# iris-ua/iris_lama

Measured on AMD Instinct MI355X. Metric: particle-scans/sec, higher is better.
Workload: dtype f64; 1 GPU; PFSlam2D 30 particles, 1080-beam synthetic corridor log (SURVEY.md 8(d)), res 0.05 m, patch 32, l2_max 0.5, GN+Cauchy(0.15), seed 42; particles=30, beams=1080, parallelism=particle-shard x1

## Files before the change

include/lama_hip.h:

```cpp
#ifndef LAMA_HIP_H
#define LAMA_HIP_H

#include <stdint.h>

#ifdef __cplusplus
extern "C" {
#endif

#define LAMA_HIP_OK 0
#define LAMA_HIP_E_INVALID (-1)
#define LAMA_HIP_E_HIP (-2)
#define LAMA_HIP_E_WINDOW (-3)
#define LAMA_HIP_E_CAPACITY (-4)
#define LAMA_HIP_E_STATE (-5)
#define LAMA_HIP_E_NUMERIC (-6)

typedef struct lama_hip_ctx lama_hip_ctx;

typedef struct lama_hip_cfg {
    uint32_t particles;
    double resolution;
    uint32_t patch_size;
    double l2_max;
    double meas_sigma;
    uint32_t max_iter;
    double truncated_ray;
    double truncated_range;
    int32_t device;
    uint32_t window_patches;
    uint32_t dm_patch_capacity;
    uint32_t occ_patch_capacity;
    uint32_t queue_capacity;
    uint32_t profile;
    uint32_t active_capacity;
    uint32_t sequential_raycast;
    uint32_t brushfire_mode;
    uint32_t brushfire_waves;
    uint32_t occupancy_policy;
    uint32_t ray_rule;
    uint32_t solver_strategy;
} lama_hip_cfg;

void lama_hip_default_cfg(lama_hip_cfg* cfg);

int32_t lama_hip_device_count(int32_t* count);

int32_t lama_hip_ctx_create(const lama_hip_cfg* cfg, lama_hip_ctx** out);
void lama_hip_ctx_destroy(lama_hip_ctx* ctx);
const char* lama_hip_last_error(const lama_hip_ctx* ctx);

int32_t lama_hip_pf_init(lama_hip_ctx* ctx, const double* pts_xyz, uint32_t n,
                         const double* sensor_origin3, const double* sensor_quat_wxyz,
                         const double* pose0);

int32_t lama_hip_pf_set_poses(lama_hip_ctx* ctx, const double* poses);
int32_t lama_hip_pf_get_poses(lama_hip_ctx* ctx, double* poses);

int32_t lama_hip_pf_scan_match(lama_hip_ctx* ctx, const double* pts_xyz, uint32_t n,
                               const double* sensor_origin3, const double* sensor_quat_wxyz,
                               double* poses_out, double* loglik_out, int32_t* iters_out);

int32_t lama_hip_pf_resample(lama_hip_ctx* ctx, const int32_t* sample_idx);

int32_t lama_hip_pf_update_maps(lama_hip_ctx* ctx, const double* pts_xyz, uint32_t n,
                                const double* sensor_origin3, const double* sensor_quat_wxyz);

#define LAMA_HIP_MAP_DISTANCE 0
#define LAMA_HIP_MAP_OCCUPANCY 1
int32_t lama_hip_pf_map_patches(lama_hip_ctx* ctx, uint32_t particle, int32_t kind, uint32_t* num_patches);
int32_t lama_hip_pf_download_map(lama_hip_ctx* ctx, uint32_t particle, int32_t kind, uint32_t cap,
                                 uint64_t* patch_ids, uint8_t* cells, uint64_t* masks, uint32_t* num_patches);

int32_t lama_hip_pf_upload_map(lama_hip_ctx* ctx, uint32_t particle, int32_t kind, uint32_t num_patches,
                               const uint64_t* patch_ids, const uint8_t* cells, const uint64_t* masks);

int32_t lama_hip_pf_update_maps_begin(lama_hip_ctx* ctx, const double* pts_xyz, uint32_t n,
// ... 128 lines not shown
```

iris_lama_amd/csrc/lama_hip.hip:

```cpp
#include "../../include/lama_hip.h"

#include <hip/hip_runtime.h>

#include <algorithm>
#include <cmath>
#include <cstdio>
#include <cstdlib>
#include <cstring>
#include <map>
#include <memory>
#include <mutex>
#include <string>
#include <vector>

#include "lama_kernels.h"
#include "lama_pgo.h"
#include "lama_map_build.h"
#include "lama_match_batch.h"
#include "../host/pgo_pattern.hpp"

using namespace lama_dev;

namespace {

// ... 151 lines not shown
    DevBuf<uint8_t> d_early; DevBuf<uint32_t> d_elist;
    Stream stream3; Event ev_alloc, ev_go, ev_early;
    bool early_ok = false;
    uint32_t early_candidates = 0;
    std::vector<double> h_ll; bool ll_valid = false;
    PinVec<uint32_t> h_hlist; DevBuf<uint32_t> d_hlist;
    uint32_t early_on = 1;
    uint32_t early_min_count = 1024;
    Stream stream2; Event ev_route, ev_heavy;
    uint32_t route_min_count = 64, route_min_events = 48, route_percent = 150, route_cap = 64;
    bool route_forced = false; uint32_t num_cus = 256;
    bool debug_tail = false, debug_window = false;
    uint32_t big_stage_pad = 0;
    DevBuf<uint64_t> d_act; DevBuf<uint32_t> d_act_count;
    DevBuf<lama_dev::RayRec> d_rrec; DevBuf<uint64_t> d_rbbox; DevBuf<lama_dev::RayChunk> d_rchunk;
    int32_t* d_err = nullptr;
    DevBuf<double> d_pts; uint32_t last_n = 0;
    PinVec<uint64_t> h_stats;
    PinVec<double> h_tfs, h_pts;
    PinVec<int32_t> h_err;
    PinVec<uint32_t> h_slow_n;
    DevBuf<double> d_tfs;
    double* d_loglik = nullptr; int32_t* d_iters = nullptr;
    DevBuf<uint8_t> d_results;
    size_t results_bytes = 0, status_off = 0, status_bytes = 0;
    PinVec<uint8_t> h_status;
    PinVec<uint8_t> h_results;
    DevBuf<int32_t> d_oldcounts;
    DevBuf<double> d_mb_pts, d_mb_tfs; DevBuf<uint32_t> d_mb_offs; DevBuf<lama_dev::MbRay> d_mb_rays;
    DevBuf<uint32_t> d_mb_table, d_mb_off, d_mb_list, d_mb_bins; DevBuf<int32_t> d_mb_slot; DevBuf<uint64_t> d_mb_meta;
    PinVec<double> h_mb_tfs; PinVec<uint32_t> h_mb_offs; PinVec<uint64_t> h_mb_meta;
    DevBuf<double> d_bposes, d_bout;
    DevBuf<double> d_msb_f64; DevBuf<uint32_t> d_msb_u32;
    PinVec<double> h_msb_f64; PinVec<uint32_t> h_msb_u32;

    double scan_reach = 0.0;
    uint32_t visit_bound = 0;
    DevBuf<uint32_t> d_scalar;
    DevBuf<lama_dev::ShipDesc> d_ship_desc; DevBuf<uint8_t> d_ship_heads;
    PinVec<lama_dev::ShipDesc> h_ship_desc; PinVec<uint8_t> h_ship_heads;
    uint32_t* d_guard = nullptr;
    Affine last_mtf; uint32_t last_first = 0, last_count = 0;
    bool last_guarded = false;
    int recover_depth = 0;
    int64_t mbx0 = 0, mbx1 = 0, mby0 = 0, mby1 = 0; bool mb_valid = false;
    bool unguarded_retry = false;
// ... 844 lines not shown
}

int32_t lama_hip_device_count(int32_t* count)
{
    int n = 0;
    hipError_t e = hipGetDeviceCount(&n);
    if (count) *count = (e == hipSuccess) ? n : 0;
    return e == hipSuccess ? LAMA_HIP_OK : LAMA_HIP_E_HIP;
}

const char* lama_hip_last_error(const lama_hip_ctx* ctx) { return ctx ? ctx->error.c_str() : "null context"; }

int32_t lama_hip_ctx_create(const lama_hip_cfg* cfg_in, lama_hip_ctx** out)
{
    if (!cfg_in || !out) return LAMA_HIP_E_INVALID;
    *out = nullptr;
    lama_hip_cfg cfg = *cfg_in;
    if (cfg.window_patches == 0) cfg.window_patches = 128;
    if (cfg.dm_patch_capacity == 0) cfg.dm_patch_capacity = 128;
    if (cfg.occ_patch_capacity == 0) cfg.occ_patch_capacity = 128;
    if (cfg.queue_capacity == 0) cfg.queue_capacity = 32768;
    if (cfg.active_capacity == 0) cfg.active_capacity = 8192;
    if (cfg.active_capacity > 8192) cfg.active_capacity = 8192;
    if (cfg.brushfire_mode > 1 || cfg.brushfire_waves > 2) return LAMA_HIP_E_INVALID;
    if (cfg.particles == 0 || cfg.patch_size != 32 || !(cfg.resolution > 0) || cfg.window_patches > (uint32_t)LAMA_HIP_MAX_WINDOW ||
        (cfg.window_patches & 7) || cfg.dm_patch_capacity > 32767 || cfg.occ_patch_capacity > 32767 ||
        cfg.queue_capacity < (uint32_t)LQ_BIG)
        return LAMA_HIP_E_INVALID;
    int ndev = 0;
    if (hipGetDeviceCount(&ndev) != hipSuccess || ndev <= 0 || cfg.device < 0 || cfg.device >= ndev) return LAMA_HIP_E_HIP;

    std::unique_ptr<lama_hip_ctx, Delete> owner(new lama_hip_ctx());
    lama_hip_ctx* c = owner.get();
    c->cfg = cfg;
    std::memset(&c->ctr, 0, sizeof(c->ctr));
    c->P = cfg.particles; c->W = cfg.window_patches; c->WC = c->W * 32;
    c->ctr.window_patches = c->W;
    c->debug_tail = std::getenv("LAMA_HIP_DEBUG_TAIL") != nullptr;
    c->debug_window = std::getenv("LAMA_HIP_DEBUG_WINDOW") != nullptr;
    {
        constexpr uint32_t CU_LDS = 160u * 1024u, GRAN = 1280u;
        const uint32_t used = (uint32_t)((sizeof(lama_dev::BfLds<LQ_BIG, RQ_BIG>) + GRAN - 1) / GRAN * GRAN);
        c->big_stage_pad = CU_LDS > used + 2u * GRAN ? CU_LDS - used - 2u * GRAN : 0u;
    }
    if (const char* rr = std::getenv("LAMA_HIP_BF_ROUTE")) {
        unsigned a = 0, b = 0, pc = 0, d = 0, e = 1;
        if (std::sscanf(rr, "%u,%u,%u,%u,%u", &a, &b, &pc, &d, &e) >= 4) { c->route_min_count = a; c->route_min_events = b; c->route_percent = pc; c->route_cap = std::min(d, 256u); c->early_on = e; c->early_min_count = 0; c->route_forced = true; }
// ... 38 lines not shown
    c->d_err = c->d_iters + P;
    c->d_slow_n = reinterpret_cast<uint32_t*>(c->d_results + slow_off);
    c->d_stats = reinterpret_cast<uint64_t*>(c->d_results + slow_off + 32);
    c->d_guard = reinterpret_cast<uint32_t*>(c->d_stats + P * 4);
    c->ms.counts = reinterpret_cast<int32_t*>(c->d_guard + P * 2);
    if (c->d_qlower.alloc(P * (size_t)cfg.queue_capacity) || c->d_qraise.alloc(P * (size_t)cfg.queue_capacity)) return LAMA_HIP_E_HIP;
    if (c->d_qsizes.alloc(P * 2) || hipMemset(c->d_qsizes, 0, P * 2 * 4)) return LAMA_HIP_E_HIP;
    if (c->d_dbg.alloc(P * 16 + (1u << 20) / 8) || hipMemset(c->d_dbg, 0, P * 16 * 8 + (1u << 20))) return LAMA_HIP_E_HIP;
    if (c->d_slow.alloc(P) || hipMemset(c->d_slow, 0, P * 4)) return LAMA_HIP_E_HIP;
    if (c->d_slow_list.alloc(4 * P) || hipMemset(c->d_slow_list, 0, 4 * P * 4)) return LAMA_HIP_E_HIP;
    if (c->d_heavy.alloc(P) || hipMemset(c->d_heavy, 0, P)) return LAMA_HIP_E_HIP;
    if (c->d_early.alloc(P) || hipMemset(c->d_early, 0, P)) return LAMA_HIP_E_HIP;
    if (c->d_elist.alloc(256) || hipMemset(c->d_elist, 0, 256 * 4)) return LAMA_HIP_E_HIP;
    if (c->d_hlist.alloc(256) || hipMemset(c->d_hlist, 0, 256 * 4)) return LAMA_HIP_E_HIP;
    if (hipStreamCreate(&c->stream2.h) || hipStreamCreate(&c->stream3.h)) return LAMA_HIP_E_HIP;
    if (hipEventCreateWithFlags(&c->ev_alloc.h, hipEventDisableTiming) || hipEventCreateWithFlags(&c->ev_early.h, hipEventDisableTiming) ||
        hipEventCreateWithFlags(&c->ev_go.h, hipEventDisableTiming) ||
        hipEventCreateWithFlags(&c->ev_route.h, hipEventDisableTiming) || hipEventCreateWithFlags(&c->ev_heavy.h, hipEventDisableTiming))
        return LAMA_HIP_E_HIP;
    if (c->d_scalar.alloc(4) || hipMemset(c->d_scalar, 0, 16)) return LAMA_HIP_E_HIP;
    if (c->d_act.alloc(P * (size_t)cfg.active_capacity)) return LAMA_HIP_E_HIP;
    if (c->d_act_count.alloc(P) || hipMemset(c->d_act_count, 0, P * 4)) return LAMA_HIP_E_HIP;
    if (c->d_tfs.alloc(P * 12) || c->d_oldcounts.alloc(P * 2)) return LAMA_HIP_E_HIP;
    if (hipDeviceSynchronize()) return LAMA_HIP_E_HIP;
    c->h_poses.assign(P * 4, 0.0);
    c->h_counts.assign(P * 2, 0);
    *out = owner.release();
    return LAMA_HIP_OK;
}

void lama_hip_ctx_destroy(lama_hip_ctx* c) { delete c; }

int32_t lama_hip_pf_set_poses(lama_hip_ctx* c, const double* poses)
{
    if (!c || !poses) return LAMA_HIP_E_INVALID;
    ENTER(c);
    HIPCHK(c, hipSetDevice(c->cfg.device));
    std::memcpy(c->h_poses.data(), poses, sizeof(double) * 4 * c->P);
    HIPCHK(c, hipMemcpyAsync(c->d_poses, c->h_poses.data(), sizeof(double) * 4 * c->P, hipMemcpyHostToDevice, c->stream));
    return LAMA_HIP_OK;
}

int32_t lama_hip_pf_get_poses(lama_hip_ctx* c, double* poses)
{
    if (!c || !poses) return LAMA_HIP_E_INVALID;
    ENTER(c);
// ... 25 lines not shown
        std::vector<int32_t> idx(c->P, 0);
        rc = permute_particles(c, idx.data());
        if (rc) return rc;
    }
    rc = check_device_errors(c, true, false);
    if (rc) return rc;
    c->initialised = true;
    return LAMA_HIP_OK;
}

int32_t lama_hip_pf_scan_match(lama_hip_ctx* c, const double* pts, uint32_t n, const double* origin3, const double* quat,
                               double* poses_out, double* loglik_out, int32_t* iters_out)
{
    if (!c || !pts || n == 0) return LAMA_HIP_E_INVALID;
    ENTER(c);
    if (!c->initialised) return fail(c, LAMA_HIP_E_STATE, "lama_hip_pf_scan_match before lama_hip_pf_init");
    HIPCHK(c, hipSetDevice(c->cfg.device));
    int32_t rc = upload_scan(c, pts, n);
    if (rc) return rc;
    const Affine mtf = moving_tf(origin3, quat);
    DevParams prm = make_params(c);
    {
        Timer t(c, &c->ctr.ms_scan_match, &c->ctr.launches_scan_match);
        if (c->max_sqdist > (uint32_t)SM_LUT) hipLaunchKernelGGL(k_scan_match<true>, dim3(c->P), dim3(SM_BLOCK), 0, c->stream, prm, c->d_pts, (int)n, mtf, c->d_loglik, c->d_iters);
        else hipLaunchKernelGGL(k_scan_match<false>, dim3(c->P), dim3(SM_BLOCK), 0, c->stream, prm, c->d_pts, (int)n, mtf, c->d_loglik, c->d_iters);
        t.stop();
    }
    HIPCHK(c, hipGetLastError());
    c->h_results.resize(c->results_bytes);
    HIPCHK(c, hipMemcpyAsync(c->h_results.data(), c->d_results, c->results_bytes, hipMemcpyDeviceToHost, c->stream));
    rc = check_device_errors(c, false, c->cfg.profile != 0, true);
    if (rc) return rc;
    const uint8_t* r = c->h_results.data();
    std::memcpy(c->h_poses.data(), r, sizeof(double) * 4 * c->P);
    if (poses_out) std::memcpy(poses_out, r, sizeof(double) * 4 * c->P);
    if (loglik_out) std::memcpy(loglik_out, r + sizeof(double) * 4 * c->P, sizeof(double) * c->P);
    if (iters_out) std::memcpy(iters_out, r + sizeof(double) * 5 * c->P, sizeof(int32_t) * c->P);
    c->h_ll.resize(c->P); std::memcpy(c->h_ll.data(), r + sizeof(double) * 4 * c->P, sizeof(double) * c->P); c->ll_valid = true;
    return LAMA_HIP_OK;
}

int32_t lama_hip_pf_resample(lama_hip_ctx* c, const int32_t* sample_idx)
{
    if (!c || !sample_idx) return LAMA_HIP_E_INVALID;
    ENTER(c);
    if (!c->initialised) return fail(c, LAMA_HIP_E_STATE, "lama_hip_pf_resample before lama_hip_pf_init");
    for (uint32_t i = 0; i < c->P; ++i)
        if (sample_idx[i] < 0 || (uint32_t)sample_idx[i] >= c->P) return fail(c, LAMA_HIP_E_INVALID, "sample_idx out of range");
    HIPCHK(c, hipSetDevice(c->cfg.device));
    c->early_ok = false;
    if (c->ll_valid) { std::vector<double> nl(c->P); for (uint32_t i = 0; i < c->P; ++i) nl[i] = c->h_ll[sample_idx[i]]; c->h_ll.swap(nl); }
    return permute_particles(c, sample_idx);
}

int32_t lama_hip_pf_update_maps_begin(lama_hip_ctx* c, const double* pts, uint32_t n, const double* origin3, const double* quat)
{
    if (!c || n == 0) return LAMA_HIP_E_INVALID;
    ENTER(c);
    if (!c->initialised) return fail(c, LAMA_HIP_E_STATE, "lama_hip_pf_update_maps before lama_hip_pf_init");
    HIPCHK(c, hipSetDevice(c->cfg.device));
    int32_t rc = upload_scan(c, pts, n);
// ... 1208 lines not shown
}

uint32_t lama_hip_counters_bytes(void) { return (uint32_t)sizeof(lama_hip_counters); }

int32_t lama_hip_get_counters_sized(lama_hip_ctx* c, void* out, uint32_t bytes)
{
    if (!c || !out) return LAMA_HIP_E_INVALID;
    lama_hip_counters full;
    const int32_t rc = lama_hip_get_counters(c, &full);
    if (rc) return rc;
    std::memcpy(out, &full, std::min<size_t>(bytes, sizeof(full)));
    return LAMA_HIP_OK;
}

int32_t lama_hip_reset_counters(lama_hip_ctx* c)
{
    if (!c) return LAMA_HIP_E_INVALID;
    ENTER(c);
    const lama_hip_counters old = c->ctr;
    std::memset(&c->ctr, 0, sizeof(c->ctr));
    c->ctr.dm_patches = old.dm_patches; c->ctr.occ_patches = old.occ_patches;
    c->ctr.brushfire_mode = old.brushfire_mode; c->ctr.brushfire_waves = old.brushfire_waves;
    c->ctr.window_patches = c->W; c->ctr.peer_access = old.peer_access;
    return LAMA_HIP_OK;
}

}
```

iris_lama_amd/csrc/lama_kernels.h:

```cpp
#pragma once
#include "lama_dev.h"

namespace lama_dev {

constexpr int SM_BLOCK = 256;
constexpr int UM_BLOCK = 64;
#ifdef LAMA_TEST_SMALL_QUEUES
constexpr int LQ_SMALL = LAMA_TEST_SMALL_QUEUES, RQ_SMALL = LAMA_TEST_SMALL_QUEUES / 4;
#else
constexpr int LQ_SMALL = 1024, RQ_SMALL = 256;
#endif
constexpr int LQ_BIG = 8192, RQ_BIG = 2048;
constexpr uint32_t BF_TW_MAX_PARTICLES = 1u << 30;

template <int CTRL, int ROW_MASK>
__device__ __forceinline__ double dpp_add(double v)
{
    const uint64_t u = (uint64_t)__double_as_longlong(v);
    const uint32_t lo = (uint32_t)__builtin_amdgcn_update_dpp(0, (int)(uint32_t)u, CTRL, ROW_MASK, 0xF, false);
    const uint32_t hi = (uint32_t)__builtin_amdgcn_update_dpp(0, (int)(uint32_t)(u >> 32), CTRL, ROW_MASK, 0xF, false);
    return v + __longlong_as_double((long long)(((uint64_t)hi << 32) | lo));
}

template <int NV>
__device__ inline void block_sum(double (&acc)[NV], double* sh , double* out )
{
    const int lane = threadIdx.x & 63, wave = threadIdx.x >> 6;
#pragma unroll
    for (int k = 0; k < NV; ++k) acc[k] = dpp_add<0xB1, 0xF>(acc[k]);
#pragma unroll
    for (int k = 0; k < NV; ++k) acc[k] = dpp_add<0x4E, 0xF>(acc[k]);
#pragma unroll
    for (int k = 0; k < NV; ++k) acc[k] = dpp_add<0x141, 0xF>(acc[k]);
#pragma unroll
    for (int k = 0; k < NV; ++k) acc[k] = dpp_add<0x140, 0xF>(acc[k]);
#pragma unroll
    for (int k = 0; k < NV; ++k) acc[k] = dpp_add<0x142, 0xA>(acc[k]);
#pragma unroll
    for (int k = 0; k < NV; ++k) acc[k] = dpp_add<0x143, 0xC>(acc[k]);
    if (lane == 63) {
#pragma unroll
        for (int k = 0; k < NV; ++k) sh[wave * NV + k] = acc[k];
    }
    __syncthreads();
    if (threadIdx.x < NV) {
        double s = sh[threadIdx.x];
        for (int w = 1; w < SM_BLOCK / 64; ++w) s += sh[w * NV + threadIdx.x];
        out[threadIdx.x] = s;
    }
    __syncthreads();
}

constexpr int NJ = 11;

constexpr int SM_NB = 5;
constexpr int SM_LUT = 512;

__device__ inline void sm_build_lut(const DevParams& prm, double* lut)
{
    for (int k = threadIdx.x; k < SM_LUT; k += SM_BLOCK) lut[k] = sqrt((double)k) * prm.resolution;
}

struct BeamCorners {
    double hx, hy, mu0, mu1;
    uint32_t off[4];
// ... 108 lines not shown
}

template <bool BIGSQ, class WT = WCauchy015>
__device__ inline void eval_beams_res(const DevParams& prm, const int16_t* dir, const sv_t* sv,
                                      const double* __restrict__ pts, int n, const Affine& tf, double (&acc)[2], const double* lut,
                                      const WT wt = WT())
{
    acc[0] = 0.0; acc[1] = 0.0;
    for (int base = 0; base < n; base += SM_NB * SM_BLOCK) {
        BeamCorners bc[SM_NB];
        sv_t cv[SM_NB][4];
        const int nb = sm_gather(prm, dir, sv, pts, n, base, tf, bc, cv);
#pragma unroll
        for (int b = 0; b < SM_NB; ++b) {
            const bool own = b < nb;
            const double d = sm_corners_finish<BIGSQ>(prm, lut, bc[b], cv[b], nullptr, nullptr);
            const double wr = d * sqrt(wt(d));
            acc[0] += own ? wr * wr : 0.0;
            acc[1] += own ? -(d * d) / prm.meas_sigma : 0.0;
        }
    }
}

struct SMShared {
    double lut[SM_LUT];
    double red[(SM_BLOCK / 64) * NJ];
    double tot[NJ];
    double tot2[NJ];
    int have_lin;
    int lin_is_final;
    Affine tf;
    SE2 state;
    double h[3];
    int ctl[2];
    double mu, v, keep[NJ];
    int reuse;
};

#ifdef LAMA_PROFILE_SM
#define SMT(k) do { const uint64_t t_ = __builtin_readcyclecounter(); smp[k] += t_ - smt; smt = t_; } while (0)
#else
#define SMT(k) do {} while (0)
#endif
template <bool BIGSQ, class WT = WCauchy015>
__device__ inline uint32_t gn_solve(const DevParams& prm, const int16_t* dir, const sv_t* sv, const double* __restrict__ pts, int n,
                                    const Affine& mtf, SMShared& sh, uint32_t& evals, const WT wt = WT(), int* numeric = nullptr)
{
#ifdef LAMA_PROFILE_SM
    uint64_t smp[4] = {0, 0, 0, 0};
    uint64_t smt = __builtin_readcyclecounter();
#endif
    const double eps1 = 1e-4, eps2 = 1e-4, tau = 1e-4;
    const bool lm = prm.strategy == 1;
    uint32_t iter = 0;
    if (threadIdx.x == 0) { sh.mu = -1.0; sh.v = 2.0; sh.reuse = 0; sh.have_lin = 0; sh.lin_is_final = 0; }
    __syncthreads();
    while (iter < prm.max_iter) {
        if (sh.have_lin) {
            ++evals;
        } else if (!sh.reuse) {
            double acc[NJ];
            {
                const Affine tf = sh.tf;
                eval_beams_jac<BIGSQ>(prm, dir, sv, pts, n, tf, acc, sh.lut, wt);
            }
            SMT(0);
            block_sum<NJ>(acc, sh.red, sh.tot);
            SMT(1);
            ++evals;
        } else {
            __syncthreads();
            if (threadIdx.x < NJ) sh.tot[threadIdx.x] = sh.keep[threadIdx.x];
            __syncthreads();
        }
        if (threadIdx.x == 0) {
            const double* t = sh.tot;
            const double g[3] = {t[6], t[7], t[8]};
            const double max_abs_g = fmax(fabs(g[0]), fmax(fabs(g[1]), fabs(g[2])));
            int stop = 0;
            sh.lin_is_final = 1;
            if (lm) for (int k = 0; k < NJ; ++k) sh.keep[k] = t[k];
            if (max_abs_g < eps1) {
                stop = 1;
            } else {
                const double A[3][3] = {{t[0], 0, 0}, {t[1], t[2], 0}, {t[3], t[4], t[5]}};
                const double mg[3] = {-g[0], -g[1], -g[2]};
                double h[3];
                if (lm) {
                    if (sh.mu < 0) sh.mu = tau * fmax(t[0], fmax(t[2], t[5]));
                    const double Au[3][3] = {{t[0] + sh.mu, t[1], t[3]}, {0, t[2] + sh.mu, t[4]}, {0, 0, t[5] + sh.mu}};
                    llt3_solve(Au, mg, h);
                } else
                ldlt3_solve(A, mg, h);
                const double max_abs_h = fmax(fabs(h[0]), fmax(fabs(h[1]), fabs(h[2])));
                if (max_abs_h < eps2) stop = 1;
                sh.h[0] = h[0]; sh.h[1] = h[1]; sh.h[2] = h[2];
                if (!stop) {
                    bool ok = true;
                    sh.state = se2_exp_mul(h, sh.state, ok);
                    if (!ok) { if (numeric) *numeric = 1; else atomicOr(prm.err, ERR_NUMERIC); }
                    sh.tf = scan_tf(sh.state, mtf);
                    sh.lin_is_final = 0;
                }
            }
            sh.ctl[0] = stop;
        }
        __syncthreads();
        SMT(2);
        if (sh.ctl[0]) break;
        double acc2[NJ];
        {
            const Affine tf = sh.tf;
            eval_beams_jac<BIGSQ>(prm, dir, sv, pts, n, tf, acc2, sh.lut, wt);
        }
        SMT(0);
        block_sum<NJ>(acc2, sh.red, sh.tot2);
        SMT(1);
        ++evals;
        if (threadIdx.x == 0) {
            const double dF = sh.tot[9] - sh.tot2[9];
            int stop = 0;
            bool invalid = !(dF > 0);
            if (lm) {
                const double* h = sh.h;
                const double* gk = sh.keep + 6;
                const double dL = 0.5 * ((h[0] * (sh.mu * h[0] - gk[0]) + h[1] * (sh.mu * h[1] - gk[1])) + h[2] * (sh.mu * h[2] - gk[2]));
                if (dL > 0.0 && dF > 0.0) {
                    const double q = 2 * (dF / dL) - 1;
                    sh.mu = sh.mu * fmax(1.0 / 3.0, 1 - q * q * q);
                    sh.v = 2.0;
                    invalid = false;
                } else {
                    sh.mu = sh.mu * sh.v; sh.v = 2 * sh.v;
                    invalid = true;
                }
                sh.reuse = invalid ? 1 : 0;
            }
            if (invalid) {
                stop = lm ? 0 : 1;
// ... 2 lines not shown
                sh.state = se2_exp_mul(mh, sh.state, ok);
                if (!ok) { if (numeric) *numeric = 1; else atomicOr(prm.err, ERR_NUMERIC); }
                sh.tf = scan_tf(sh.state, mtf);
                sh.have_lin = 0;
            } else {
                for (int k = 0; k < NJ; ++k) sh.tot[k] = sh.tot2[k];
                sh.have_lin = 1;
                sh.lin_is_final = 1;
            }
            sh.ctl[1] = stop;
        }
        ++iter;
        __syncthreads();
        SMT(3);
        if (sh.ctl[1]) break;
    }
#ifdef LAMA_PROFILE_SM
    if (threadIdx.x == 0) for (int k = 0; k < 4; ++k) prm.dbg[8 * blockIdx.x + k] = smp[k];
#endif
    return iter;
}
#undef SMT

template <bool BIGSQ>
__global__ __launch_bounds__(SM_BLOCK) __attribute__((amdgpu_num_vgpr(128))) void k_scan_match(DevParams prm, const double* __restrict__ pts, int n, Affine mtf,
                                                          double* __restrict__ loglik_out, int32_t* __restrict__ iters_out)
{
    __shared__ SMShared sh;
    const int p = blockIdx.x;
    const PV pv_ = pview_w(prm, p);
    const int16_t* dir = pv_.dm_dir;
    const sv_t* sv = pv_.dm_sv;
    if (threadIdx.x == 0) {
        const double* q = prm.poses + 4 * p;
        sh.state = SE2{cload_f64(q), cload_f64(q + 1), cload_f64(q + 2), cload_f64(q + 3)};
        sh.tf = scan_tf(sh.state, mtf);
        sh.ctl[0] = 0; sh.ctl[1] = 0;
    }
    sm_build_lut(prm, sh.lut);
    __syncthreads();
    uint32_t evals = 0;
    const uint32_t iter = gn_solve<BIGSQ>(prm, dir, sv, pts, n, mtf, sh, evals);
    double loglik;
    if (sh.lin_is_final) {
        loglik = sh.tot[10];
    } else {
        double a2[2];
        {
            const Affine tf = sh.tf;
            eval_beams_res<BIGSQ>(prm, dir, sv, pts, n, tf, a2, sh.lut);
        }
        block_sum<2>(a2, sh.red, sh.tot2);
        loglik = sh.tot2[1];
    }
    ++evals;
    if (threadIdx.x == 0) {
        double* q = prm.poses + 4 * p;
        q[0] = sh.state.c; q[1] = sh.state.s; q[2] = sh.state.tx; q[3] = sh.state.ty;
        loglik_out[p] = loglik;
        iters_out[p] = (int32_t)iter;
        prm.stats[4 * p + 0] = iter;
        prm.stats[4 * p + 1] = evals;
    }
}

template <bool BIGSQ>
__global__ __launch_bounds__(SM_BLOCK) void k_match_solve(DevParams prm, int particle, const double* __restrict__ pts, int n, Affine mtf,
                                                           double* __restrict__ pose_io, double* __restrict__ out7, int32_t* __restrict__ iters_out,
                                                           int do_solve)
{
    __shared__ SMShared sh;
    const PV pv_ = pview_w(prm, particle);
    const int16_t* dir = pv_.dm_dir;
    const sv_t* sv = pv_.dm_sv;
    if (threadIdx.x == 0) {
        sh.state = SE2{cload_f64(pose_io), cload_f64(pose_io + 1), cload_f64(pose_io + 2), cload_f64(pose_io + 3)};
        sh.tf = scan_tf(sh.state, mtf);
        sh.ctl[0] = 0; sh.ctl[1] = 0;
    }
    sm_build_lut(prm, sh.lut);
    __syncthreads();
    uint32_t evals = 0;
// ... 1999 lines not shown
```

iris_lama_amd/ffi.py:

```python
import ctypes as C
import math
import os
import sys

import numpy as np

_HERE = os.path.dirname(os.path.abspath(__file__))
HIP_LIB = os.path.join(_HERE, "lib", "liblama_hip.so")
HIP_LIB_WIDE = os.path.join(_HERE, "lib", "liblama_hip_wide.so")
HOST_LIB = os.path.join(_HERE, "lib", "liblama_host.so")
_PRODUCT_HOST_LIB = HOST_LIB

MAP_DISTANCE, MAP_OCCUPANCY = 0, 1

DIST_T = np.dtype([("obstacle", "<i2", (3,)), ("sqdist", "<u2"), ("valid", "u1"), ("queued", "u1")])
FREQ_T = np.dtype([("occupied", "<u2"), ("visited", "<u2")])


class LamaError(RuntimeError):
    pass


class HipCfg(C.Structure):
    _fields_ = [("particles", C.c_uint32), ("resolution", C.c_double), ("patch_size", C.c_uint32),
                ("l2_max", C.c_double), ("meas_sigma", C.c_double), ("max_iter", C.c_uint32),
                ("truncated_ray", C.c_double), ("truncated_range", C.c_double), ("device", C.c_int32),
                ("window_patches", C.c_uint32), ("dm_patch_capacity", C.c_uint32),
                ("occ_patch_capacity", C.c_uint32), ("queue_capacity", C.c_uint32), ("profile", C.c_uint32),
                ("active_capacity", C.c_uint32), ("sequential_raycast", C.c_uint32), ("brushfire_mode", C.c_uint32),
                ("brushfire_waves", C.c_uint32), ("occupancy_policy", C.c_uint32), ("ray_rule", C.c_uint32),
                ("solver_strategy", C.c_uint32)]


class HipCounters(C.Structure):
    _fields_ = [("ms_scan_match", C.c_double), ("launches_scan_match", C.c_uint64),
                ("ms_update_maps", C.c_double), ("launches_update_maps", C.c_uint64),
                ("ms_raycast", C.c_double), ("launches_raycast", C.c_uint64),
                ("ms_brushfire", C.c_double), ("launches_brushfire", C.c_uint64),
                ("ms_resample", C.c_double), ("launches_resample", C.c_uint64),
                ("gn_iterations", C.c_uint64), ("gn_evals", C.c_uint64), ("ray_cells", C.c_uint64),
                ("bf_cells", C.c_uint64), ("dm_patches", C.c_uint64), ("occ_patches", C.c_uint64),
                ("ms_eval_batch", C.c_double), ("launches_eval_batch", C.c_uint64), ("arena_growths", C.c_uint64), ("window_shifts", C.c_uint64), ("wrap_guard_scans", C.c_uint64),
                ("brushfire_mode", C.c_uint32), ("brushfire_waves", C.c_uint32),
                ("sequential_raycast_scans", C.c_uint64), ("parallel_raycast_scans", C.c_uint64),
                ("brushfire_handovers", C.c_uint32), ("replay_handovers", C.c_uint32),
                ("window_patches", C.c_uint32), ("window_growths", C.c_uint32),
                ("bf_longest_chain_sum", C.c_uint64), ("bf_longest_chain_last", C.c_uint64), ("brushfire_early", C.c_uint64), ("brushfire_routed", C.c_uint64),
                ("pool_growths", C.c_uint64), ("resample_clones", C.c_uint64), ("resample_bytes", C.c_uint64),
                ("hbm_bytes_allocated", C.c_uint64), ("hbm_bytes_used", C.c_uint64), ("hbm_bytes_total", C.c_uint64),
                ("peer_access", C.c_uint32), ("struct_bytes", C.c_uint32), ("peer_copy_ms", C.c_double), ("peer_copy_bytes", C.c_uint64)]

    def as_dict(self):
        return {n: getattr(self, n) for n, _ in self._fields_}


HIP_SYMBOLS = [
    "lama_hip_default_cfg", "lama_hip_device_count", "lama_hip_ctx_create", "lama_hip_ctx_destroy",
    "lama_hip_last_error", "lama_hip_pf_init", "lama_hip_pf_set_poses", "lama_hip_pf_get_poses",
    "lama_hip_pf_scan_match", "lama_hip_pf_resample", "lama_hip_pf_update_maps", "lama_hip_pf_map_patches",
    "lama_hip_pf_download_map", "lama_hip_pf_upload_map", "lama_hip_match_batch", "lama_hip_pf_export_particle",
    "lama_hip_pf_import_particle", "lama_hip_get_counters", "lama_hip_get_counters_sized", "lama_hip_counters_bytes", "lama_hip_reset_counters",
    "lama_hip_map_add_obstacles", "lama_hip_match_solve", "lama_hip_eval_batch", "lama_hip_map_sample_likelihood",
    "lama_hip_pgo_create", "lama_hip_pgo_destroy", "lama_hip_pgo_last_error", "lama_hip_pgo_linearize",
    "lama_hip_pf_patch_ids", "lama_hip_pf_delete_patches", "lama_hip_pf_update_maps_begin", "lama_hip_sync", "lama_hip_ctx_device",
    "lama_hip_pf_map_checksums", "lama_hip_match_eval", "lama_hip_match_cell_distances", "lama_hip_match_solve_with",
    "lama_hip_blob_alloc", "lama_hip_blob_free", "lama_hip_blob_copy", "lama_hip_pf_export_particles", "lama_hip_pf_import_particles",
    "lama_hip_pgo_pattern", "lama_hip_pgo_set_poses", "lama_hip_pgo_get_poses", "lama_hip_pgo_linearize_system",
    "lama_hip_pgo_try_step", "lama_hip_pgo_accept",
    "lama_hip_map_integrate_scans", "lama_hip_map_occupied_cells",
    "lama_hip_match_solve_batch",
]

_hip = None
_hip_wide = None


def _torch_runtime_first():
    if "torch" not in sys.modules and not os.environ.get("LAMA_NO_TORCH_PRELOAD"):
        try:
            import importlib.util
            if importlib.util.find_spec("torch") is not None:
                import torch
        except Exception:
            pass


def hip_lib(wide=False):
    global _hip, _hip_wide
    if wide:
        if _hip_wide is None:
            if not os.path.exists(HIP_LIB_WIDE):
                raise LamaError(f"{HIP_LIB_WIDE} is missing: run `python -c 'import __graft_entry__ as g; g.build()'`. There is no CPU fallback.")
            _torch_runtime_first()
# ... 67 lines not shown
        L.lama_hip_get_counters_sized.argtypes = [vp, vp, u32]
        L.lama_hip_counters_bytes.argtypes = []
        L.lama_hip_counters_bytes.restype = C.c_uint32
        L.lama_hip_reset_counters.argtypes = [vp]
        L.lama_hip_map_add_obstacles.argtypes = [vp, u32, vp, u32]
        L.lama_hip_match_solve.argtypes = [vp, u32, vp, u32, vp, vp, vp, vp, vp, i32]
        L.lama_hip_eval_batch.argtypes = [vp, u32, vp, u32, vp, vp, vp, u32, vp, vp]
        L.lama_hip_pf_patch_ids.argtypes = [vp, u32, i32, u32, vp, vp]
        L.lama_hip_pf_delete_patches.argtypes = [vp, u32, vp, u32, vp]
        L.lama_hip_map_sample_likelihood.argtypes = [vp, u32, vp, u32, vp, vp, C.c_double, vp, u32, u32, vp]
        L.lama_hip_match_eval.argtypes = [vp, u32, vp, u32, vp, vp, vp, vp, vp]
        L.lama_hip_match_cell_distances.argtypes = [vp, u32, vp, u32, vp, vp, vp, vp]
        L.lama_hip_match_solve_with.argtypes = [vp, u32, vp, u32, vp, vp, vp, vp, vp, i32, u32]
        has_mb = hasattr(L, "lama_hip_map_integrate_scans")
        if has_mb:
            L.lama_hip_map_integrate_scans.argtypes = [vp, u32, u32, vp, vp, vp, vp, vp, u32]
            L.lama_hip_map_occupied_cells.argtypes = [vp, u32, u32, vp, vp]
        has_msb = hasattr(L, "lama_hip_match_solve_batch")
        if has_msb:
            L.lama_hip_match_solve_batch.argtypes = [vp, u32, vp, vp, vp, vp, vp, vp, vp, i32, i32, C.c_double, vp, vp, vp]
        has_cks = hasattr(L, "lama_hip_pf_map_checksums")
        if has_cks:
            L.lama_hip_pf_map_checksums.argtypes = [vp, i32, vp]
        has_pgo = hasattr(L, "lama_hip_pgo_create")
        if has_pgo:
            L.lama_hip_pgo_create.argtypes = [i32, u32, vp, vp, vp, vp, u32, vp]
            L.lama_hip_pgo_destroy.argtypes = [vp]
            L.lama_hip_pgo_destroy.restype = None
            L.lama_hip_pgo_last_error.argtypes = [vp]
            L.lama_hip_pgo_last_error.restype = C.c_char_p
            L.lama_hip_pgo_linearize.argtypes = [vp, vp, vp, vp, vp, vp, vp, vp]
            L.lama_hip_pgo_pattern.argtypes = [vp, vp, vp, vp]
            L.lama_hip_pgo_set_poses.argtypes = [vp, vp]
            L.lama_hip_pgo_get_poses.argtypes = [vp, vp]
            L.lama_hip_pgo_linearize_system.argtypes = [vp, vp, vp, vp, vp, vp]
            L.lama_hip_pgo_try_step.argtypes = [vp, vp, vp, vp]
            L.lama_hip_pgo_accept.argtypes = [vp]
        for s in HIP_SYMBOLS:
            if s.startswith("lama_hip_pgo_") and not has_pgo:
                continue
            if s == "lama_hip_pf_map_checksums" and not has_cks:
                continue
            if s in ("lama_hip_map_integrate_scans", "lama_hip_map_occupied_cells") and not has_mb:
                continue
            if s == "lama_hip_match_solve_batch" and not has_msb:
                continue
            if s not in ("lama_hip_default_cfg", "lama_hip_ctx_destroy", "lama_hip_last_error", "lama_hip_pgo_destroy",
                         "lama_hip_pgo_last_error"):
                getattr(L, s).restype = i32


def _p(a):
    return a.ctypes.data_as(C.c_void_p) if a is not None else None


_IDQ = np.array([1.0, 0.0, 0.0, 0.0])
_Z3 = np.zeros(3)


MAP_BUILD_FULL, MAP_BUILD_PRUNE = 1, 2
ROBUST_KINDS = {"unit": 0, "tukey": 1, "tdist": 2, "cauchy": 3, "huber": 4}
ROBUST_STORED = 0x100
E_NUMERIC = -6


def pack_scans(scans):
    if isinstance(scans, tuple) and len(scans) == 2 and not (hasattr(scans[1], "ndim") and np.ndim(scans[1]) == 2):
        pts = np.ascontiguousarray(scans[0], dtype=np.float64)
# ... 70 lines not shown

    def init(self, pts, pose0, origin=None, quat=None):
        pts, origin, quat = self._scan(pts, origin, quat)
        pose0 = np.ascontiguousarray(pose0, dtype=np.float64)
        self._chk(self.L.lama_hip_pf_init(self.h, _p(pts), len(pts), _p(origin), _p(quat), _p(pose0)))

    def set_poses(self, poses):
        poses = np.ascontiguousarray(poses, dtype=np.float64)
        assert poses.shape == (self.P, 4)
        self._chk(self.L.lama_hip_pf_set_poses(self.h, _p(poses)))

    def get_poses(self):
        out = np.zeros((self.P, 4))
        self._chk(self.L.lama_hip_pf_get_poses(self.h, _p(out)))
        return out

    def scan_match(self, pts, origin=None, quat=None):
        pts, origin, quat = self._scan(pts, origin, quat)
        poses = np.zeros((self.P, 4))
        ll = np.zeros(self.P)
        it = np.zeros(self.P, dtype=np.int32)
        self._chk(self.L.lama_hip_pf_scan_match(self.h, _p(pts), len(pts), _p(origin), _p(quat), _p(poses), _p(ll), _p(it)))
        return poses, ll, it

    def resample(self, idx):
        idx = np.ascontiguousarray(idx, dtype=np.int32)
        assert idx.shape == (self.P,)
        self._chk(self.L.lama_hip_pf_resample(self.h, _p(idx)))

    def update_maps(self, pts, origin=None, quat=None):
        pts, origin, quat = self._scan(pts, origin, quat)
        self._chk(self.L.lama_hip_pf_update_maps(self.h, _p(pts), len(pts), _p(origin), _p(quat)))

    def download_map(self, particle, kind):
        n = C.c_uint32(0)
        self._chk(self.L.lama_hip_pf_map_patches(self.h, particle, kind, C.byref(n)))
        n = n.value
        ids = np.zeros(n, dtype=np.uint64)
        dt = DIST_T if kind == MAP_DISTANCE else FREQ_T
        cells = np.zeros((n, 1024), dtype=dt)
        masks = np.zeros((n, 16), dtype=np.uint64)
        got = C.c_uint32(0)
        self._chk(self.L.lama_hip_pf_download_map(self.h, particle, kind, n, _p(ids), _p(cells), _p(masks), C.byref(got)))
        assert got.value == n
        return {int(ids[k]): (cells[k], masks[k]) for k in range(n)}

# ... 1090 lines not shown
```

Before: 16850 particle-scans/s.

## Add wide 1024-thread scan-match kernel for small particle counts

Result: slower. 16590 particle-scans/s (-1.5%).

```diff
diff --git a/include/lama_hip.h b/include/lama_hip.h
--- a/include/lama_hip.h
+++ b/include/lama_hip.h
@@ -39,6 +39,7 @@
     uint32_t occupancy_policy;
     uint32_t ray_rule;
     uint32_t solver_strategy;
+    uint32_t scan_match_form;
 } lama_hip_cfg;
 
 void lama_hip_default_cfg(lama_hip_cfg* cfg);
@@ -52,6 +53,8 @@
 int32_t lama_hip_pf_init(lama_hip_ctx* ctx, const double* pts_xyz, uint32_t n,
                          const double* sensor_origin3, const double* sensor_quat_wxyz,
                          const double* pose0);
+
+int32_t lama_hip_debug_scan_match(lama_hip_ctx* ctx, double* chi2, uint64_t* wide_launches);
 
 int32_t lama_hip_pf_set_poses(lama_hip_ctx* ctx, const double* poses);
 int32_t lama_hip_pf_get_poses(lama_hip_ctx* ctx, double* poses);
diff --git a/iris_lama_amd/csrc/lama_hip.hip b/iris_lama_amd/csrc/lama_hip.hip
--- a/iris_lama_amd/csrc/lama_hip.hip
+++ b/iris_lama_amd/csrc/lama_hip.hip
@@ -197,6 +197,8 @@
     PinVec<uint32_t> h_slow_n;
     DevBuf<double> d_tfs;
     double* d_loglik = nullptr; int32_t* d_iters = nullptr;
+    DevBuf<double> d_chi2;
+    uint64_t wide_scan_matches = 0;
     DevBuf<uint8_t> d_results;
     size_t results_bytes = 0, status_off = 0, status_bytes = 0;
     PinVec<uint8_t> h_status;
@@ -1087,7 +1089,7 @@
     if (cfg.queue_capacity == 0) cfg.queue_capacity = 32768;
     if (cfg.active_capacity == 0) cfg.active_capacity = 8192;
     if (cfg.active_capacity > 8192) cfg.active_capacity = 8192;
-    if (cfg.brushfire_mode > 1 || cfg.brushfire_waves > 2) return LAMA_HIP_E_INVALID;
+    if (cfg.brushfire_mode > 1 || cfg.brushfire_waves > 2 || cfg.scan_match_form > 2) return LAMA_HIP_E_INVALID;
     if (cfg.particles == 0 || cfg.patch_size != 32 || !(cfg.resolution > 0) || cfg.window_patches > (uint32_t)LAMA_HIP_MAX_WINDOW ||
         (cfg.window_patches & 7) || cfg.dm_patch_capacity > 32767 || cfg.occ_patch_capacity > 32767 ||
         cfg.queue_capacity < (uint32_t)LQ_BIG)
@@ -1172,6 +1174,7 @@
     if (c->d_act.alloc(P * (size_t)cfg.active_capacity)) return LAMA_HIP_E_HIP;
     if (c->d_act_count.alloc(P) || hipMemset(c->d_act_count, 0, P * 4)) return LAMA_HIP_E_HIP;
     if (c->d_tfs.alloc(P * 12) || c->d_oldcounts.alloc(P * 2)) return LAMA_HIP_E_HIP;
+    if (c->d_chi2.alloc(P) || hipMemset(c->d_chi2, 0, P * 8)) return LAMA_HIP_E_HIP;
     if (hipDeviceSynchronize()) return LAMA_HIP_E_HIP;
     c->h_poses.assign(P * 4, 0.0);
     c->h_counts.assign(P * 2, 0);
@@ -1243,8 +1246,14 @@
     DevParams prm = make_params(c);
     {
         Timer t(c, &c->ctr.ms_scan_match, &c->ctr.launches_scan_match);
-        if (c->max_sqdist > (uint32_t)SM_LUT) hipLaunchKernelGGL(k_scan_match<true>, dim3(c->P), dim3(SM_BLOCK), 0, c->stream, prm, c->d_pts, (int)n, mtf, c->d_loglik, c->d_iters);
-        else hipLaunchKernelGGL(k_scan_match<false>, dim3(c->P), dim3(SM_BLOCK), 0, c->stream, prm, c->d_pts, (int)n, mtf, c->d_loglik, c->d_iters);
+        const bool wide = c->cfg.scan_match_form == 2 || (c->cfg.scan_match_form == 0 && c->P <= SMW_MAX_PARTICLES);
+        const bool bigsq = c->max_sqdist > (uint32_t)SM_LUT;
+        double* const chi2 = c->d_chi2;
+        if (wide && bigsq) hipLaunchKernelGGL((k_scan_match<true, SMW_BLOCK>), dim3(c->P), dim3(SMW_BLOCK), 0, c->stream, prm, c->d_pts, (int)n, mtf, c->d_loglik, c->d_iters, chi2);
+        else if (wide) hipLaunchKernelGGL((k_scan_match<false, SMW_BLOCK>), dim3(c->P), dim3(SMW_BLOCK), 0, c->stream, prm, c->d_pts, (int)n, mtf, c->d_loglik, c->d_iters, chi2);
+        else if (bigsq) hipLaunchKernelGGL((k_scan_match<true, SM_BLOCK>), dim3(c->P), dim3(SM_BLOCK), 0, c->stream, prm, c->d_pts, (int)n, mtf, c->d_loglik, c->d_iters, chi2);
+        else hipLaunchKernelGGL((k_scan_match<false, SM_BLOCK>), dim3(c->P), dim3(SM_BLOCK), 0, c->stream, prm, c->d_pts, (int)n, mtf, c->d_loglik, c->d_iters, chi2);
+        if (wide) c->wide_scan_matches += 1;
         t.stop();
     }
     HIPCHK(c, hipGetLastError());
@@ -1258,6 +1267,19 @@
     if (loglik_out) std::memcpy(loglik_out, r + sizeof(double) * 4 * c->P, sizeof(double) * c->P);
     if (iters_out) std::memcpy(iters_out, r + sizeof(double) * 5 * c->P, sizeof(int32_t) * c->P);
     c->h_ll.resize(c->P); std::memcpy(c->h_ll.data(), r + sizeof(double) * 4 * c->P, sizeof(double) * c->P); c->ll_valid = true;
+    return LAMA_HIP_OK;
+}
+
+int32_t lama_hip_debug_scan_match(lama_hip_ctx* c, double* chi2, uint64_t* wide_launches)
+{
+    if (!c) return LAMA_HIP_E_INVALID;
+    ENTER(c);
+    if (chi2) {
+        HIPCHK(c, hipSetDevice(c->cfg.device));
+        HIPCHK(c, hipMemcpyAsync(chi2, c->d_chi2, sizeof(double) * c->P, hipMemcpyDeviceToHost, c->stream));
+        HIPCHK(c, hipStreamSynchronize(c->stream));
+    }
+    if (wide_launches) *wide_launches = c->wide_scan_matches;
     return LAMA_HIP_OK;
 }
 
@@ -2512,7 +2534,8 @@
     c->ctr.dm_patches = old.dm_patches; c->ctr.occ_patches = old.occ_patches;
     c->ctr.brushfire_mode = old.brushfire_mode; c->ctr.brushfire_waves = old.brushfire_waves;
     c->ctr.window_patches = c->W; c->ctr.peer_access = old.peer_access;
-    return LAMA_HIP_OK;
-}
-
-}
+    c->wide_scan_matches = 0;
+    return LAMA_HIP_OK;
+}
+
+}
diff --git a/iris_lama_amd/csrc/lama_kernels.h b/iris_lama_amd/csrc/lama_kernels.h
--- a/iris_lama_amd/csrc/lama_kernels.h
+++ b/iris_lama_amd/csrc/lama_kernels.h
@@ -22,10 +22,11 @@
     return v + __longlong_as_double((long long)(((uint64_t)hi << 32) | lo));
 }
 
-template <int NV>
+template <int NV, int BLOCK = SM_BLOCK>
 __device__ inline void block_sum(double (&acc)[NV], double* sh , double* out )
 {
     const int lane = threadIdx.x & 63, wave = threadIdx.x >> 6;
+    if (BLOCK == SM_BLOCK || threadIdx.x < SM_BLOCK) {
 #pragma unroll
     for (int k = 0; k < NV; ++k) acc[k] = dpp_add<0xB1, 0xF>(acc[k]);
 #pragma unroll
@@ -41,6 +42,7 @@
     if (lane == 63) {
 #pragma unroll
         for (int k = 0; k < NV; ++k) sh[wave * NV + k] = acc[k];
+    }
     }
     __syncthreads();
     if (threadIdx.x < NV) {
@@ -195,6 +197,108 @@
     }
 }
 
+constexpr int SMW_BLOCK = 1024, SMW_Q = SMW_BLOCK / SM_BLOCK;
+constexpr int SMW_NX = 5;
+constexpr uint32_t SMW_MAX_PARTICLES = 64;
+
+template <bool BIGSQ>
+__device__ inline double smw_beam(const DevParams& prm, const int16_t* __restrict__ dir, const sv_t* __restrict__ sv,
+                                  const double* __restrict__ pts, int i, const Affine& tf, const double* lut, double* hx, double* hy,
+                                  double* gx, double* gy)
+{
+    BeamCorners bc;
+    sm_corners_begin(prm, tf, pts[3 * i], pts[3 * i + 1], pts[3 * i + 2], bc);
+    int16_t sl[4];
+#pragma unroll
+    for (int c = 0; c < 4; ++c) sl[c] = dir[bc.off[c]];
+#pragma unroll
+    for (int c = 0; c < 4; ++c) {
+        const bool have = ((bc.okm >> c) & 1u) && sl[c] >= 0;
+        bc.off[c] = have ? (uint32_t)sl[c] * 1024u + bc.ci[c] : 0u;
+        if (!have) bc.okm &= ~(1u << c);
+    }
+    sv_t cv[4];
+#pragma unroll
+    for (int c = 0; c < 4; ++c) cv[c] = sv[bc.off[c]];
+    *hx = bc.hx; *hy = bc.hy;
+    return sm_corners_finish<BIGSQ>(prm, lut, bc, cv, gx, gy);
+}
+
+template <bool BIGSQ, class WT = WCauchy015>
+__device__ inline void eval_beams_jac_wide(const DevParams& prm, const int16_t* dir, const sv_t* sv, const double* __restrict__ pts, int n,
+                                           const Affine& tf, double (&acc)[NJ], const double* lut, double* xch ,
+                                           const WT wt = WT())
+{
+    const int t = (int)threadIdx.x & (SM_BLOCK - 1), q = (int)threadIdx.x / SM_BLOCK;
+#pragma unroll
+    for (int k = 0; k < NJ; ++k) acc[k] = 0.0;
+    for (int base = 0; base < n; base += SMW_BLOCK) {
+        double f[SMW_NX] = {0.0, 0.0, 0.0, 0.0, 0.0};
+        const int i = base + (int)threadIdx.x;
+        if (i < n) {
+            double hx, hy, gx, gy;
+            double r = smw_beam<BIGSQ>(prm, dir, sv, pts, i, tf, lut, &hx, &hy, &gx, &gy);
+            f[4] = -(r * r) / prm.meas_sigma;
+            const double w = sqrt(wt(r));
+            r *= w;
+            f[0] = gx * w; f[1] = gy * w; f[2] = (gy * hx - gx * hy) * w; f[3] = r;
+        }
+        if (base) __syncthreads();
+        if (q > 0) {
+#pragma unroll
+            for (int k = 0; k < SMW_NX; ++k) xch[(k * (SMW_Q - 1) + (q - 1)) * SM_BLOCK + t] = f[k];
+        }
+        __syncthreads();
+        if (q == 0) {
+#pragma unroll
+            for (int qq = 0; qq < SMW_Q; ++qq) {
+                if (qq > 0) {
+#pragma unroll
+                    for (int k = 0; k < SMW_NX; ++k) f[k] = xch[(k * (SMW_Q - 1) + (qq - 1)) * SM_BLOCK + t];
+                }
+                const bool own = base + qq * SM_BLOCK + t < n;
+                const double j0 = f[0], j1 = f[1], j2 = f[2], r = f[3];
+                acc[10] += own ? f[4] : 0.0;
+                acc[0] += own ? j0 * j0 : 0.0; acc[1] += own ? j1 * j0 : 0.0; acc[2] += own ? j1 * j1 : 0.0;
+                acc[3] += own ? j2 * j0 : 0.0; acc[4] += own ? j2 * j1 : 0.0; acc[5] += own ? j2 * j2 : 0.0;
+                acc[6] += own ? j0 * r : 0.0;  acc[7] += own ? j1 * r : 0.0;  acc[8] += own ? j2 * r : 0.0;
+                acc[9] += own ? r * r : 0.0;
+            }
+        }
+    }
+}
+
+template <bool BIGSQ, class WT = WCauchy015>
+__device__ inline void eval_beams_res_wide(const DevParams& prm, const int16_t* dir, const sv_t* sv, const double* __restrict__ pts, int n,
+                                           const Affine& tf, double (&acc)[2], const double* lut, double* xch, const WT wt = WT())
+{
+    const int t = (int)threadIdx.x & (SM_BLOCK - 1), q = (int)threadIdx.x / SM_BLOCK;
+    acc[0] = 0.0; acc[1] = 0.0;
+    for (int base = 0; base < n; base += SMW_BLOCK) {
+        double f[2] = {0.0, 0.0};
+        const int i = base + (int)threadIdx.x;
+        if (i < n) {
+            double hx, hy;
+            const double d = smw_beam<BIGSQ>(prm, dir, sv, pts, i, tf, lut, &hx, &hy, nullptr, nullptr);
+            const double wr = d * sqrt(wt(d));
+            f[0] = wr * wr;
+            f[1] = -(d * d) / prm.meas_sigma;
+        }
+        if (base) __syncthreads();
+        if (q > 0) { xch[(q - 1) * SM_BLOCK + t] = f[0]; xch[((SMW_Q - 1) + (q - 1)) * SM_BLOCK + t] = f[1]; }
+        __syncthreads();
+        if (q == 0) {
+#pragma unroll
+            for (int qq = 0; qq < SMW_Q; ++qq) {
+                if (qq > 0) { f[0] = xch[(qq - 1) * SM_BLOCK + t]; f[1] = xch[((SMW_Q - 1) + (qq - 1)) * SM_BLOCK + t]; }
+                const bool own = base + qq * SM_BLOCK + t < n;
+                acc[0] += own ? f[0] : 0.0;
+                acc[1] += own ? f[1] : 0.0;
+            }
+        }
+    }
+}
+
 struct SMShared {
     double lut[SM_LUT];
     double red[(SM_BLOCK / 64) * NJ];
@@ -215,9 +319,10 @@
 #else
 #define SMT(k) do {} while (0)
 #endif
-template <bool BIGSQ, class WT = WCauchy015>
+template <bool BIGSQ, class WT = WCauchy015, int BLOCK = SM_BLOCK>
 __device__ inline uint32_t gn_solve(const DevParams& prm, const int16_t* dir, const sv_t* sv, const double* __restrict__ pts, int n,
-                                    const Affine& mtf, SMShared& sh, uint32_t& evals, const WT wt = WT(), int* numeric = nullptr)
+                                    const Affine& mtf, SMShared& sh, uint32_t& evals, const WT wt = WT(), int* numeric = nullptr,
+                                    double* xch = nullptr)
 {
 #ifdef LAMA_PROFILE_SM
     uint64_t smp[4] = {0, 0, 0, 0};
@@ -235,10 +340,11 @@
             double acc[NJ];
             {
                 const Affine tf = sh.tf;
-                eval_beams_jac<BIGSQ>(prm, dir, sv, pts, n, tf, acc, sh.lut, wt);
+                if constexpr (BLOCK == SM_BLOCK) eval_beams_jac<BIGSQ>(prm, dir, sv, pts, n, tf, acc, sh.lut, wt);
+                else eval_beams_jac_wide<BIGSQ>(prm, dir, sv, pts, n, tf, acc, sh.lut, xch, wt);
             }
             SMT(0);
-            block_sum<NJ>(acc, sh.red, sh.tot);
+            block_sum<NJ, BLOCK>(acc, sh.red, sh.tot);
             SMT(1);
             ++evals;
         } else {
@@ -284,10 +390,11 @@
         double acc2[NJ];
         {
             const Affine tf = sh.tf;
-            eval_beams_jac<BIGSQ>(prm, dir, sv, pts, n, tf, acc2, sh.lut, wt);
+            if constexpr (BLOCK == SM_BLOCK) eval_beams_jac<BIGSQ>(prm, dir, sv, pts, n, tf, acc2, sh.lut, wt);
+            else eval_beams_jac_wide<BIGSQ>(prm, dir, sv, pts, n, tf, acc2, sh.lut, xch, wt);
         }
         SMT(0);
-        block_sum<NJ>(acc2, sh.red, sh.tot2);
+        block_sum<NJ, BLOCK>(acc2, sh.red, sh.tot2);
         SMT(1);
         ++evals;
         if (threadIdx.x == 0) {
@@ -336,11 +443,17 @@
 }
 #undef SMT
 
-template <bool BIGSQ>
-__global__ __launch_bounds__(SM_BLOCK) __attribute__((amdgpu_num_vgpr(128))) void k_scan_match(DevParams prm, const double* __restrict__ pts, int n, Affine mtf,
-                                                          double* __restrict__ loglik_out, int32_t* __restrict__ iters_out)
+template <bool BIGSQ, int BLOCK = SM_BLOCK>
+__global__ __launch_bounds__(BLOCK) __attribute__((amdgpu_num_vgpr(128))) void k_scan_match(DevParams prm, const double* __restrict__ pts, int n, Affine mtf,
+                                                          double* __restrict__ loglik_out, int32_t* __restrict__ iters_out,
+                                                          double* __restrict__ chi2_out)
 {
     __shared__ SMShared sh;
+    double* xch = nullptr;
+    if constexpr (BLOCK != SM_BLOCK) {
+        __shared__ double xbuf[SMW_NX * (SMW_Q - 1) * SM_BLOCK];
+        xch = xbuf;
+    }
     const int p = blockIdx.x;
     const PV pv_ = pview_w(prm, p);
     const int16_t* dir = pv_.dm_dir;
@@ -354,24 +467,26 @@
     sm_build_lut(prm, sh.lut);
     __syncthreads();
     uint32_t evals = 0;
-    const uint32_t iter = gn_solve<BIGSQ>(prm, dir, sv, pts, n, mtf, sh, evals);
-    double loglik;
+    const uint32_t iter = gn_solve<BIGSQ, WCauchy015, BLOCK>(prm, dir, sv, pts, n, mtf, sh, evals, WCauchy015(), nullptr, xch);
+    double loglik, chi2;
     if (sh.lin_is_final) {
-        loglik = sh.tot[10];
+        loglik = sh.tot[10]; chi2 = sh.tot[9];
     } else {
         double a2[2];
         {
             const Affine tf = sh.tf;
-            eval_beams_res<BIGSQ>(prm, dir, sv, pts, n, tf, a2, sh.lut);
-        }
-        block_sum<2>(a2, sh.red, sh.tot2);
-        loglik = sh.tot2[1];
+            if constexpr (BLOCK == SM_BLOCK) eval_beams_res<BIGSQ>(prm, dir, sv, pts, n, tf, a2, sh.lut);
+            else eval_beams_res_wide<BIGSQ>(prm, dir, sv, pts, n, tf, a2, sh.lut, xch);
+        }
+        block_sum<2, BLOCK>(a2, sh.red, sh.tot2);
+        loglik = sh.tot2[1]; chi2 = sh.tot2[0];
     }
     ++evals;
     if (threadIdx.x == 0) {
         double* q = prm.poses + 4 * p;
         q[0] = sh.state.c; q[1] = sh.state.s; q[2] = sh.state.tx; q[3] = sh.state.ty;
         loglik_out[p] = loglik;
+        chi2_out[p] = chi2;
         iters_out[p] = (int32_t)iter;
         prm.stats[4 * p + 0] = iter;
         prm.stats[4 * p + 1] = evals;
diff --git a/iris_lama_amd/ffi.py b/iris_lama_amd/ffi.py
--- a/iris_lama_amd/ffi.py
+++ b/iris_lama_amd/ffi.py
@@ -29,7 +29,7 @@
                 ("occ_patch_capacity", C.c_uint32), ("queue_capacity", C.c_uint32), ("profile", C.c_uint32),
                 ("active_capacity", C.c_uint32), ("sequential_raycast", C.c_uint32), ("brushfire_mode", C.c_uint32),
                 ("brushfire_waves", C.c_uint32), ("occupancy_policy", C.c_uint32), ("ray_rule", C.c_uint32),
-                ("solver_strategy", C.c_uint32)]
+                ("solver_strategy", C.c_uint32), ("scan_match_form", C.c_uint32)]
 
 
 class HipCounters(C.Structure):
@@ -68,7 +68,7 @@
     "lama_hip_pgo_pattern", "lama_hip_pgo_set_poses", "lama_hip_pgo_get_poses", "lama_hip_pgo_linearize_system",
     "lama_hip_pgo_try_step", "lama_hip_pgo_accept",
     "lama_hip_map_integrate_scans", "lama_hip_map_occupied_cells",
-    "lama_hip_match_solve_batch",
+    "lama_hip_match_solve_batch", "lama_hip_debug_scan_match",
 ]
 
 _hip = None
@@ -182,6 +182,9 @@
         has_cks = hasattr(L, "lama_hip_pf_map_checksums")
         if has_cks:
             L.lama_hip_pf_map_checksums.argtypes = [vp, i32, vp]
+        has_dsm = hasattr(L, "lama_hip_debug_scan_match")
+        if has_dsm:
+            L.lama_hip_debug_scan_match.argtypes = [vp, vp, vp]
         has_pgo = hasattr(L, "lama_hip_pgo_create")
         if has_pgo:
             L.lama_hip_pgo_create.argtypes = [i32, u32, vp, vp, vp, vp, u32, vp]
@@ -204,6 +207,8 @@
             if s in ("lama_hip_map_integrate_scans", "lama_hip_map_occupied_cells") and not has_mb:
                 continue
             if s == "lama_hip_match_solve_batch" and not has_msb:
+                continue
+            if s == "lama_hip_debug_scan_match" and not has_dsm:
                 continue
             if s not in ("lama_hip_default_cfg", "lama_hip_ctx_destroy", "lama_hip_last_error", "lama_hip_pgo_destroy",
                          "lama_hip_pgo_last_error"):
@@ -320,6 +325,12 @@
         it = np.zeros(self.P, dtype=np.int32)
         self._chk(self.L.lama_hip_pf_scan_match(self.h, _p(pts), len(pts), _p(origin), _p(quat), _p(poses), _p(ll), _p(it)))
         return poses, ll, it
+
+    def scan_match_debug(self):
+        chi2 = np.zeros(self.P)
+        wide = C.c_uint64(0)
+        self._chk(self.L.lama_hip_debug_scan_match(self.h, _p(chi2), C.byref(wide)))
+        return chi2, wide.value
 
     def resample(self, idx):
         idx = np.ascontiguousarray(idx, dtype=np.int32)
```
